# SingleRust/single-algebra

Hardware: AMD Instinct MI355X
Metric: sparse_pca_fit_transform_algorithmic_throughput (higher is better)
Workload: dtype f32

## Files before the change

single-algebra_amd/csrc/spmm_tiled.hip:

```cpp
#include <cstdio>
#include <cstdlib>
#include <cstring>

#include <rocprim/rocprim.hpp>

#include "kernels.h"
#include "spmm_dq.h"

namespace sapca {
namespace k {

namespace {

constexpr int WAVE = 64;
constexpr int LDS_TOTAL = 160 * 1024;

struct Ent { uint32_t off; float val; };
struct EntD { uint32_t off; uint32_t pad; double val; };
template <typename VT> struct EntOf { typedef Ent type; };
template <> struct EntOf<double> { typedef EntD type; };

inline int grid_for(int64_t work_items, int block, int cap = 8192) {
  int64_t g = (work_items + block - 1) / block;
  if (g < 1) g = 1;
  if (g > cap) g = cap;
  return (int)g;
}

typedef float v4f __attribute__((ext_vector_type(4)));
typedef float v4f_a4 __attribute__((ext_vector_type(4), aligned(4)));

template <int N, int THREADS>
__device__ __forceinline__ void load_regs(v4f (&r)[N], const char* src, int bytes) {
#pragma unroll
  for (int i = 0; i < N; ++i)
    r[i] = *reinterpret_cast<const v4f*>(src + min((i * THREADS + (int)threadIdx.x) * 16, bytes - 16));
}
template <int N, int THREADS>
__device__ __forceinline__ void store_regs(const v4f (&r)[N], char* dst, int capacity) {
#pragma unroll
  for (int i = 0; i < N; ++i) {
    const int b = (i * THREADS + (int)threadIdx.x) * 16;
    if ((i + 1) * THREADS * 16 <= capacity || b + 16 <= capacity) *reinterpret_cast<v4f*>(dst + b) = r[i];
  }
}

template <typename VT>
__global__ void split_reduce_kernel(const VT* __restrict__ part, int nsplit, int64_t rows, int ldo, int ncols,
                                    const VT* __restrict__ cvec, VT* __restrict__ out, int ldy) {
  const int64_t total = rows * ldo;
  int64_t i = (int64_t)blockIdx.x * blockDim.x + threadIdx.x;
  const int64_t stride = (int64_t)gridDim.x * blockDim.x;
  for (; i < total; i += stride) {
    const int j = (int)(i % ldo);
    if (j >= ncols) continue;
    VT s = 0;
    for (int sp = 0; sp < nsplit; ++sp) s += part[(int64_t)sp * total + i];
    out[(i / ldo) * ldy + j] = s - (cvec ? cvec[j] : (VT)0);
  }
}

__global__ void split_reduce_rows_kernel(const float* __restrict__ part, int nsplit, int64_t slab_stride, int64_t rows, int ldo, int ncols,
                                         float* __restrict__ out, int ldy) {
  const int64_t total = rows * ldo;
  int64_t i = (int64_t)blockIdx.x * blockDim.x + threadIdx.x;
  const int64_t stride = (int64_t)gridDim.x * blockDim.x;
  for (; i < total; i += stride) {
    const int j = (int)(i % ldo);
    if (j >= ncols) continue;
    float s = 0;
    for (int sp = 0; sp < nsplit; ++sp) s += part[(int64_t)sp * slab_stride + i];
    out[(i / ldo) * ldy + j] = s;
  }
}

#ifndef SAPCA_QWAVES
#define SAPCA_QWAVES 16
#endif
constexpr int QGROUPS = 4, QLANES = WAVE / QGROUPS, QWAVES = SAPCA_QWAVES, QTHREADS = QWAVES * WAVE;
constexpr int Q_TILE_BYTES = 80 * 1024;
constexpr int Q_MAX_TILES_RUNS = 16384;
constexpr int q_stage_bytes(int tile_bytes) { return LDS_TOTAL - tile_bytes - 1024; }
constexpr int QBLOCK_ROWS = 1024;
constexpr int Q_BLOCK_QUADS = QBLOCK_ROWS / 4;
constexpr int ENT_SLACK = 4 * WAVE;
constexpr int q_rows_per_group(int ldp) { return (ldp == 64 ? 128 : 64) / QWAVES; }
__host__ __device__ inline int q_steps(int longest) { return kOddSteps ? longest : (longest + 1) & ~1; }
__host__ __device__ inline int q_first(int wave, int nquads) { return wave * nquads / QWAVES; }

// ... 91 lines not shown
    for (int off = 1; off < WAVE; off <<= 1) {
      const uint32_t y = __shfl_up(inc, off);
      if (lane >= off) inc += y;
    }
#pragma unroll
    for (int off = WAVE / 2; off > 0; off >>= 1) raw += __shfl_xor(raw, off);
    __syncthreads();
    if (lane == WAVE - 1) wave_total[q / WAVE] = inc;
    if (lane == 0) raw_part[q / WAVE] = (uint32_t)raw;
    __syncthreads();
    for (int w = 0; w < q / WAVE; ++w) inc += wave_total[w];
    scan[q] = inc;
    __syncthreads();
    if (quad_off && q < nquads) quad_off[((int64_t)rb * Q_BLOCK_QUADS + q) * nct + ct] = inc - padded;
    if (q < QWAVES) {
      const int first_quad = q_first(q, nquads);
      wave_off[chunk * QWAVES + q] = first_quad > 0 ? scan[first_quad - 1] : 0u;
    }
    if (q == Q_BLOCK_QUADS - 1) {
      chunk_size[chunk] = inc;
      if (raw_size) {
        uint32_t total = 0;
        for (int w = 0; w < Q_BLOCK_QUADS / WAVE; ++w) total += raw_part[w];
        raw_size[chunk] = total;
      }
    }
  }
}

template <typename VT>
__global__ void __launch_bounds__(256)
quad_fill_kernel(const int64_t* __restrict__ ptr, const int32_t* __restrict__ idx, const VT* __restrict__ val,
                 int64_t rows, const int32_t* __restrict__ blk_row0, const uint32_t* __restrict__ perm, int nrb, int nct,
                 float inv_nct, int ldp_bytes, const int64_t* __restrict__ chunk_off, const uint32_t* __restrict__ quad_off,
                 typename EntOf<VT>::type* __restrict__ ent) {
  typedef typename EntOf<VT>::type E;
  extern __shared__ uint32_t cnt_all[];
  const int wave = threadIdx.x / WAVE, lane = threadIdx.x & (WAVE - 1);
  uint32_t* cnt = cnt_all + (size_t)wave * nct;
  const int64_t sp = (int64_t)blockIdx.x * 4 + wave;
  if (sp >= rows) return;
  const int64_t r = perm ? (int64_t)perm[sp] : sp;
  int lo = 0, hi = nrb;
  while (hi - lo > 1) {
    const int mid = (lo + hi) >> 1;
    if ((int64_t)blk_row0[mid] <= sp) lo = mid; else hi = mid;
  }
  const int rb = lo;
  const int lr = (int)(sp - blk_row0[rb]);
  const int qd = lr >> 2;
  const uint32_t g = (uint32_t)(lr & 3);
  const int64_t* __restrict__ coff = chunk_off + (int64_t)rb * nct;
  const uint32_t* __restrict__ qoff = quad_off + ((int64_t)rb * Q_BLOCK_QUADS + qd) * nct;
  const int64_t block_base = coff[0];
  for (int t = lane; t < nct; t += WAVE) cnt[t] = (uint32_t)(coff[t] - block_base) + qoff[t] + g;
  __builtin_amdgcn_wave_barrier();
  const int64_t e0 = ptr[r], e1 = ptr[r + 1];
  E* __restrict__ out = ent + block_base;
  for (int64_t eb = e0; eb < e1; eb += 8 * WAVE) {
    int c[8];
    VT v[8];
#pragma unroll
    for (int u = 0; u < 8; ++u) {
      const int64_t e = eb + u * WAVE + lane;
      c[u] = e < e1 ? idx[e] : -1;
      v[u] = e < e1 ? val[e] : (VT)0;
    }
#pragma unroll
    for (int u = 0; u < 8; ++u) {
      if (c[u] >= 0) {
        int i, t;
        divmod_small(c[u], nct, inv_nct, i, t);
        E x = E();
        x.off = (uint32_t)i * (uint32_t)ldp_bytes;
        x.val = v[u];
        out[atomicAdd(&cnt[t], 4u)] = x;
      }
      __builtin_amdgcn_wave_barrier();
    }
  }
}

constexpr int QF_CAP_MIN = 4096, QF_CAP_MAX = 6144;
template <typename VT>
__device__ __forceinline__ void quad_fill_staged_one(int qi, uint32_t* qf_lds, const int64_t* __restrict__ ptr, const int32_t* __restrict__ idx,
                                                     const VT* __restrict__ val, const int32_t* __restrict__ seg,
                                                     const int32_t* __restrict__ blk_row0, const uint32_t* __restrict__ perm, int nct, int cap,
                                                     float inv_nct, int ldp_bytes, const int64_t* __restrict__ chunk_off,
                                                     const uint32_t* __restrict__ quad_off, typename EntOf<VT>::type* __restrict__ ent) {
  typedef typename EntOf<VT>::type E;
  constexpr int EW = (int)sizeof(E) / 4;
  E* stage = reinterpret_cast<E*>(qf_lds);
  int64_t* gofs = reinterpret_cast<int64_t*>(qf_lds + EW * cap);
  uint32_t* lofs = qf_lds + EW * cap + 2 * nct;
  uint32_t* cnt_all = lofs + nct + 1;
  const int rb = qi / Q_BLOCK_QUADS, qd = qi % Q_BLOCK_QUADS;
  const int row0 = blk_row0[rb], nrows = blk_row0[rb + 1] - row0;
  if (4 * qd >= nrows) return;
  const int wave = threadIdx.x / WAVE, lane = threadIdx.x & (WAVE - 1);
  const int qrows = min(4, nrows - 4 * qd);
  const int64_t s0 = (int64_t)row0 + 4 * qd;
  int64_t rowof[4];
#pragma unroll
  for (int g = 0; g < 4; ++g) rowof[g] = g < qrows ? (perm ? (int64_t)perm[s0 + g] : s0 + g) : 0;
  const int64_t* __restrict__ coff = chunk_off + (int64_t)rb * nct;
  const uint32_t* __restrict__ qoff = quad_off + ((int64_t)rb * Q_BLOCK_QUADS + qd) * nct;
  for (int t = threadIdx.x; t < nct; t += 256) {
    int mx = 0;
    for (int g = 0; g < qrows; ++g) {
      const int32_t* sg = seg + rowof[g] * (nct + 1);
      mx = max(mx, sg[t + 1] - sg[t]);
    }
    lofs[t + 1] = (uint32_t)q_steps(mx) * 4u;
    gofs[t] = coff[t] + (int64_t)qoff[t];
    for (int g = 0; g < 4; ++g) cnt_all[g * nct + t] = 0;
  }
  if (threadIdx.x == 0) lofs[0] = 0;
  __syncthreads();
  if (wave == 0) {
    uint32_t carry = 0;
    for (int t0 = 0; t0 < nct; t0 += WAVE) {
      const int t = t0 + lane;
      const uint32_t v = t < nct ? lofs[t + 1] : 0u;
      uint32_t x = v;
#pragma unroll
      for (int off = 1; off < WAVE; off <<= 1) {
        const uint32_t y = __shfl_up(x, off);
        if (lane >= off) x += y;
      }
      if (t < nct) lofs[t + 1] = carry + x;
      carry += __shfl(x, WAVE - 1);
    }
  }
  __syncthreads();
  const uint32_t total = lofs[nct];
  const bool staged = total <= (uint32_t)cap;
  if (staged) {
    uint64_t* z = reinterpret_cast<uint64_t*>(stage);
    for (uint32_t i = threadIdx.x; i < total * (EW / 2); i += 256) z[i] = 0;
  } else {
    if (wave < qrows) {
      const int32_t* sg = seg + rowof[wave] * (nct + 1);
      for (int t = lane; t < nct; t += WAVE) {
        const uint32_t steps = (lofs[t + 1] - lofs[t]) / 4u;
        E* dst = ent + gofs[t];
        for (uint32_t k = (uint32_t)(sg[t + 1] - sg[t]); k < steps; ++k) dst[k * 4u + wave] = E();
      }
    } else {
      for (int t = lane; t < nct; t += WAVE) {
        const uint32_t steps = (lofs[t + 1] - lofs[t]) / 4u;
        E* dst = ent + gofs[t];
        for (uint32_t k = 0; k < steps; ++k) dst[k * 4u + wave] = E();
      }
    }
  }
  __syncthreads();
  if (wave < qrows) {
    const int64_t r = rowof[wave];
    const int64_t e0 = ptr[r], e1 = ptr[r + 1];
    uint32_t* cnt = cnt_all + (size_t)wave * nct;
    for (int64_t eb = e0; eb < e1; eb += 8 * WAVE) {
      int c[8];
      VT v[8];
#pragma unroll
      for (int u = 0; u < 8; ++u) {
        const int64_t e = eb + u * WAVE + lane;
        c[u] = e < e1 ? idx[e] : -1;
        v[u] = e < e1 ? val[e] : (VT)0;
      }
#pragma unroll
      for (int u = 0; u < 8; ++u) {
        if (c[u] >= 0) {
          int i, t;
          divmod_small(c[u], nct, inv_nct, i, t);
          E x = E();
          x.off = (uint32_t)i * (uint32_t)ldp_bytes;
          x.val = v[u];
          const uint32_t k = atomicAdd(&cnt[t], 1u);
          if (staged) stage[lofs[t] + k * 4u + (uint32_t)wave] = x;
          else ent[gofs[t] + k * 4u + (uint32_t)wave] = x;
        }
        __builtin_amdgcn_wave_barrier();
      }
    }
  }
  if (!staged) return;
  __syncthreads();
  for (int t = wave; t < nct; t += 4) {
    const uint32_t lo = lofs[t], n = lofs[t + 1] - lo;
    E* dst = ent + gofs[t];
    for (uint32_t j = lane; j < n; j += WAVE) dst[j] = stage[lo + j];
  }
}

template <typename VT>
__global__ void __launch_bounds__(256)
quad_fill_staged_kernel(const int64_t* __restrict__ ptr, const int32_t* __restrict__ idx, const VT* __restrict__ val,
                        const int32_t* __restrict__ seg, const int32_t* __restrict__ blk_row0,
                        const uint32_t* __restrict__ perm, int nct, int cap, float inv_nct,
                        int ldp_bytes, const int64_t* __restrict__ chunk_off, const uint32_t* __restrict__ quad_off,
                        typename EntOf<VT>::type* __restrict__ ent, int nquads_all) {
  extern __shared__ __attribute__((aligned(16))) uint32_t qf_lds[];
  for (int qi = blockIdx.x; qi < nquads_all; qi += gridDim.x) {
    quad_fill_staged_one<VT>(qi, qf_lds, ptr, idx, val, seg, blk_row0, perm, nct, cap, inv_nct, ldp_bytes, chunk_off, quad_off, ent);
    __syncthreads();
  }
}

__global__ void tile_index_mod_kernel(const int64_t* __restrict__ ptr, const int32_t* __restrict__ idx,
                                      const uint64_t* __restrict__ packed, int64_t rows, int nct, float inv_nct,
                                      int32_t* __restrict__ seg) {
  const int64_t total = rows * (int64_t)(nct + 1);
  int64_t o = (int64_t)blockIdx.x * blockDim.x + threadIdx.x;
  const int64_t stride = (int64_t)gridDim.x * blockDim.x;
  for (; o < total; o += stride) {
    const int64_t r = o / (nct + 1);
    const int t = (int)(o - r * (nct + 1));
    const int64_t e0 = ptr[r], e1 = ptr[r + 1];
    int64_t lo = e0, hi = e1;
    while (lo < hi) {
      const int64_t mid = (lo + hi) >> 1;
      int q, tm;
      divmod_small(packed ? (int)(packed[mid] >> 32) : idx[mid], nct, inv_nct, q, tm);
      if (tm < t) lo = mid + 1; else hi = mid;
    }
    seg[o] = (int32_t)(lo - e0);
  }
}

__global__ void at_stats_index_kernel(const int64_t* __restrict__ ptr, const uint64_t* __restrict__ packed, int64_t rows,
                                      int nct, float inv_nct, double* __restrict__ sum, double* __restrict__ sumsq,
                                      int32_t* __restrict__ seg) {
  const int lane = threadIdx.x & (WAVE - 1);
  const int64_t wave = ((int64_t)blockIdx.x * blockDim.x + threadIdx.x) / WAVE;
  const int64_t nwaves = (int64_t)gridDim.x * blockDim.x / WAVE;
  for (int64_t r = wave; r < rows; r += nwaves) {
    const int64_t e0 = ptr[r], e1 = ptr[r + 1];
    int32_t* sg = seg + r * (nct + 1);
    double a = 0, b = 0;
    int carry = -1;
    for (int64_t eb = e0; eb < e1; eb += WAVE) {
      const int64_t e = eb + lane;
      const bool valid = e < e1;
      int t = nct;
      if (valid) {
        const uint64_t pv = packed[e];
        const double v = (double)__uint_as_float((uint32_t)pv);
        a += v;
        b += v * v;
        int q;
        divmod_small((int)(pv >> 32), nct, inv_nct, q, t);
      }
      int tprev = __shfl_up(t, 1);
      if (lane == 0) tprev = carry;
      if (valid || e == e1)
        for (int tt = tprev + 1; tt <= t; ++tt) sg[tt] = (int32_t)(e - e0);
      carry = __shfl(t, WAVE - 1);
    }
    if (((e1 - e0) & (WAVE - 1)) == 0)
      for (int tt = carry + 1 + lane; tt <= nct; tt += WAVE) sg[tt] = (int32_t)(e1 - e0);
#pragma unroll
    for (int off = WAVE / 2; off > 0; off >>= 1) {
      a += __shfl_xor(a, off);
      b += __shfl_xor(b, off);
    }
    if (lane == 0) {
      sum[r] = a;
      if (sumsq) sumsq[r] = b;
    }
  }
}

__global__ void row_len_iota_kernel(const int64_t* __restrict__ ptr, int64_t rows, uint32_t* __restrict__ len,
                                    uint32_t* __restrict__ iota) {
  const int64_t r = (int64_t)blockIdx.x * blockDim.x + threadIdx.x;
  if (r < rows) {
    len[r] = (uint32_t)(ptr[r + 1] - ptr[r]);
    iota[r] = (uint32_t)r;
  }
}

__global__ void __launch_bounds__(256)
natural_quad_slots_kernel(const int64_t* __restrict__ ptr, int64_t rows, unsigned long long* __restrict__ out) {
  __shared__ unsigned long long red[4];
  unsigned long long acc = 0;
  const int64_t nq = (rows + 3) / 4;
  for (int64_t qd = (int64_t)blockIdx.x * blockDim.x + threadIdx.x; qd < nq; qd += (int64_t)gridDim.x * blockDim.x) {
    int64_t mx = 0;
// ... 846 lines not shown
          psum[(int64_t)t * n + row] = a;
          psq[(int64_t)t * n + row] = b;
        }
      }
    }
    q0 = q1;
  }
}

__global__ void __launch_bounds__(1024)
atd_stats_reduce_kernel(const double* __restrict__ psum, const double* __restrict__ psq, int64_t n, int nct,
                        double* __restrict__ sum, double* __restrict__ sumsq) {
  __shared__ double pa[16][64], pb[16][64];
  const int lane = threadIdx.x & 63, grp = threadIdx.x >> 6;
  const int64_t c = (int64_t)blockIdx.x * 64 + lane;
  const int per = (nct + 15) / 16;
  double a = 0, b = 0;
  if (c < n)
    for (int t = grp * per; t < min(nct, (grp + 1) * per); ++t) {
      a += psum[(int64_t)t * n + c];
      b += psq[(int64_t)t * n + c];
    }
  pa[grp][lane] = a;
  pb[grp][lane] = b;
  __syncthreads();
  if (grp == 0 && c < n) {
    double x = 0, y = 0;
    for (int g = 0; g < 16; ++g) {
      x += pa[g][lane];
      y += pb[g][lane];
    }
    sum[c] = x;
    sumsq[c] = y;
  }
}

}

namespace {
struct AtDirectSrc {
  const CsrView<float>* A;
  const uint16_t* cnt16;
  int64_t n2;
  DevBuf* scratch;
  double* stats;
  const uint32_t* bnd;
  int64_t nrb_nat;
  const std::vector<int32_t>* blk_nat;
  bool slots_done = false;
};

void float_blocks(int64_t n, int64_t nrb, std::vector<int32_t>& blk, float& scale) {
  scale = (float)nrb / (float)n;
  auto block_of = [&](int64_t c) { return (int64_t)(int)((float)(int)c * scale); };
  while (block_of(n - 1) > nrb - 1) scale = std::nextafterf(scale, 0.0f);
  blk.assign((size_t)nrb + 1, (int32_t)n);
  int64_t b = 0;
  blk[0] = 0;
  for (int64_t c = 0; c < n; ++c) {
    const int64_t bc = block_of(c);
    while (b < bc) blk[(size_t)++b] = (int32_t)c;
  }
  while (b < nrb) blk[(size_t)++b] = (int32_t)n;
}

int dq_block_rows(int64_t op_rows) {
  static const int dq_rows_env = dbg_env("SAPCA_DQ_BLOCK_ROWS") ? atoi(dbg_env("SAPCA_DQ_BLOCK_ROWS")) : 0;
  return dq_rows_env == 512 || dq_rows_env == 1024 ? dq_rows_env : (op_rows >= 1024 * 16 ? 1024 : 512);
}
void natural_partition(int64_t op_rows, int nct, int block_rows, int64_t& nrb, int& nsplit) {
  nrb = (op_rows + block_rows - 1) / block_rows;
  nsplit = 1;
  if (nrb >= 192) {
    nrb = round_up(nrb, 256);
  } else {
    static const int split_wgs_env = dbg_env("SAPCA_SPLIT_WGS") ? atoi(dbg_env("SAPCA_SPLIT_WGS")) : 0;
    const int64_t split_wgs = split_wgs_env > 0 ? split_wgs_env : (block_rows > 512 ? 256 : 512);
    nsplit = (int)std::min<int64_t>(nct, std::max<int64_t>(1, split_wgs / nrb));
    const int64_t nrb_fit = split_wgs / nsplit;
    if (nrb_fit >= nrb && nrb_fit <= op_rows) nrb = nrb_fit;
  }
}

inline unsigned qf_grid(int64_t nquads) {
#ifdef SAPCA_QF_WGS
  const int64_t wgs = SAPCA_QF_WGS;
#else
  const int64_t wgs = nquads;
#endif
  return (unsigned)std::max<int64_t>(1, std::min<int64_t>(nquads, wgs));
}

template <typename VT>
bool build_tiled_t(const CsrView<VT>& S, int ldp_elems, TiledOp& op, TiledBuffers& buf, hipStream_t s,
                   bool rows_tile_major, const uint64_t* packed_rows, bool seg_ready,
                   const AtDirectSrc* direct = nullptr) {
  typedef typename EntOf<VT>::type E;
  constexpr bool f32 = sizeof(VT) == 4;
  const int ldp = ldp_elems * (int)sizeof(VT) / 4;
  SAPCA_CHECK(ldp_elems == 64, SAPCA_ERR_ARG, "tiled sweep: panels must have 64 columns");
  op = TiledOp();
  if (!f32 && packed_rows) return false;
  if (S.rows == 0 || S.cols == 0 || S.nnz == 0) return false;
  const int64_t op_rows = S.rows, op_cols = S.cols;
  const int tile_bytes = Q_TILE_BYTES;
  const int tc = tile_bytes / (ldp * 4);
  if (packed_rows && !rows_tile_major) return false;
  const int nct = (int)((op_cols + tc - 1) / tc);
  const int waves = QWAVES;
  const bool dq_candidate = f32 && ldp == 64 && dbg_env("SAPCA_NO_DQ") == nullptr;
  const int block_rows = dq_candidate ? dq_block_rows(op_rows) : QWAVES * QGROUPS * q_rows_per_group(ldp);
  const int stage_cap = q_stage_bytes(tile_bytes) / (int)sizeof(E) - WAVE;
  int64_t nrb = 0;
  int nsplit = 1;
  natural_partition(op_rows, nct, block_rows, nrb, nsplit);
  if (op_cols >= (1 << 24) || nct > (rows_tile_major ? Q_MAX_TILES_RUNS : 4096)) return false;
  const float inv_nct = 1.0f / (float)nct;
  int32_t* d_seg = nullptr;
  if (direct && !(f32 && rows_tile_major && dq_candidate && tc <= 32 * ATD_MASK_WORDS && block_rows <= QBLOCK_ROWS))
    return false;
  if (!direct) {
    d_seg = buf.seg.as<int32_t>((size_t)S.rows * (nct + 1));
    if (rows_tile_major && seg_ready) {
    } else if (rows_tile_major) {
      hipLaunchKernelGGL(tile_index_mod_kernel, dim3(grid_for(S.rows * (int64_t)(nct + 1), 256, 16384)), dim3(256), 0, s,
                         S.ptr, S.idx, packed_rows, S.rows, nct, inv_nct, d_seg);
    } else {
      hipLaunchKernelGGL(tile_hist_kernel, dim3(grid_for(S.rows, 4, 8192)), dim3(256), (size_t)4 * nct * sizeof(uint32_t), s,
                         S.ptr, S.idx, S.rows, nct, inv_nct, d_seg);
    }
  }
  uint32_t* d_perm = nullptr;
  std::vector<uint32_t> sorted_len;
  bool sort_rows = dbg_env("SAPCA_NO_ROWSORT") == nullptr;
  int64_t* pinned = static_cast<int64_t*>(buf.host.ensure((size_t)(8 + 65536 + 2) * sizeof(int64_t)));
  bool speculate = false;
  bool rows_in_disorder = false;
  if (sort_rows && dbg_env("SAPCA_ROWSORT_ALWAYS") == nullptr) {
    unsigned long long* d_slots = reinterpret_cast<unsigned long long*>(buf.misc.as<int64_t>(8)) + 4;
    if (!(direct && direct->slots_done)) {
      SAPCA_HIP(hipMemsetAsync(d_slots, 0, sizeof(unsigned long long), s));
      hipLaunchKernelGGL(natural_quad_slots_kernel, dim3(grid_for((S.rows + 3) / 4, 256, 1024)), dim3(256), 0, s, S.ptr, S.rows, d_slots);
    }
    SAPCA_HIP(hipMemcpyAsync(pinned, d_slots, sizeof(unsigned long long), hipMemcpyDeviceToHost, s));
    speculate = true;
    sort_rows = false;
  }
  auto sort_now = [&] {
    uint32_t* d_len = buf.lens.as<uint32_t>((size_t)2 * S.rows);
    uint32_t* d_len_sorted = d_len + S.rows;
    uint32_t* d_iota = buf.perm.as<uint32_t>((size_t)2 * S.rows);
    d_perm = d_iota + S.rows;
    hipLaunchKernelGGL(row_len_iota_kernel, dim3(grid_for(S.rows, 256, 1 << 30)), dim3(256), 0, s, S.ptr, S.rows, d_len, d_iota);
    size_t sb = 0;
    SAPCA_HIP(rocprim::radix_sort_pairs_desc(nullptr, sb, d_len, d_len_sorted, d_iota, d_perm, (size_t)S.rows, 0u, 32u, s));
    char* tmp = static_cast<char*>(buf.tmp.ensure(sb + 256));
    SAPCA_HIP(rocprim::radix_sort_pairs_desc(tmp, sb, d_len, d_len_sorted, d_iota, d_perm, (size_t)S.rows, 0u, 32u, s));
    sorted_len.resize((size_t)S.rows);
    SAPCA_HIP(hipMemcpyAsync(sorted_len.data(), d_len_sorted, sorted_len.size() * sizeof(uint32_t), hipMemcpyDeviceToHost, s));
    SAPCA_HIP(hipStreamSynchronize(s));
  };
  if (sort_rows) sort_now();
  int tiles_per_split = 0;
  int64_t nchunks = 0, max_chunk = 0, total = 0;
  int32_t* d_blk = nullptr;
  int64_t mid_row0 = -1;
  uint8_t* d_steps = nullptr;
  uint32_t* d_wave_off = nullptr;
  uint32_t* d_quad_off = nullptr;
  int64_t* d_chunk = nullptr;
  int64_t* d_raw = nullptr;
  for (int attempt = 0;; ++attempt) {
    tiles_per_split = (nct + nsplit - 1) / nsplit;
    nsplit = (nct + tiles_per_split - 1) / tiles_per_split;
    std::vector<int32_t> blk;
    if (sort_rows) {
      const double budget = (double)S.nnz / (double)nrb;
      blk.push_back(0);
      double acc = 0;
      int in_block = 0;
      for (int64_t r = 0; r < op_rows; ++r) {
        acc += sorted_len[(size_t)r];
        ++in_block;
        const bool last = r + 1 == op_rows;
        if (last || in_block == block_rows || acc >= budget * (double)blk.size()) {
          blk.push_back((int32_t)(r + 1));
          in_block = 0;
        }
      }
      nrb = (int64_t)blk.size() - 1;
    } else if (direct && direct->bnd && nrb == direct->nrb_nat) {
      blk = *direct->blk_nat;
    } else {
      blk.resize((size_t)nrb + 1);
      for (int64_t b = 0; b <= nrb; ++b) blk[(size_t)b] = (int32_t)(op_rows * b / nrb);
    }
    nchunks = nrb * nct;
    mid_row0 = blk[(size_t)(nrb / 2)];
    d_blk = buf.blk.as<int32_t>((size_t)nrb + 1);
    d_steps = buf.steps.as<uint8_t>((size_t)nchunks * Q_BLOCK_QUADS * 2);
    d_wave_off = buf.wave_off.as<uint32_t>((size_t)nchunks * waves);
    d_quad_off = buf.run.as<uint32_t>((size_t)nchunks * Q_BLOCK_QUADS);
    d_chunk = buf.chunk_off.as<int64_t>((size_t)nchunks + 1);
    if (blk.size() <= 2 * 65536) {
      std::memcpy(pinned + 8, blk.data(), blk.size() * sizeof(int32_t));
      SAPCA_HIP(hipMemcpyAsync(d_blk, pinned + 8, blk.size() * sizeof(int32_t), hipMemcpyHostToDevice, s));
    } else {
      SAPCA_HIP(hipMemcpyAsync(d_blk, blk.data(), blk.size() * sizeof(int32_t), hipMemcpyHostToDevice, s));
    }
    if (direct) {
      d_raw = buf.rank.as<int64_t>((size_t)nchunks + 1);
      hipLaunchKernelGGL(quad_count_kernel, dim3((unsigned)(nrb * ((nct + QC_TILES - 1) / QC_TILES))), dim3(Q_BLOCK_QUADS), 0, s, d_seg, d_blk, d_perm, nct,
                         reinterpret_cast<uint16_t*>(d_steps), (uint32_t*)nullptr, d_wave_off, d_chunk, direct->cnt16, direct->n2, d_raw);
    } else
      hipLaunchKernelGGL(quad_count_kernel, dim3((unsigned)(nrb * ((nct + QC_TILES - 1) / QC_TILES))), dim3(Q_BLOCK_QUADS), 0, s, d_seg, d_blk, d_perm, nct,
                         reinterpret_cast<uint16_t*>(d_steps), d_quad_off, d_wave_off, d_chunk);
    int64_t* d_max = buf.misc.as<int64_t>(8);
    launch_small_scan(d_chunk, d_raw, nchunks, d_max, s);
    int64_t* host = pinned + 1;
    SAPCA_HIP(hipMemcpyAsync(host, d_max, (direct ? 7 : 2) * sizeof(int64_t), hipMemcpyDeviceToHost, s));
    SAPCA_HIP(hipStreamSynchronize(s));
    if (direct) rows_in_disorder = host[6] != 0;
    if (speculate) {
      speculate = false;
      if ((double)(unsigned long long)pinned[0] > 1.10 * (double)S.nnz) {
        sort_rows = true;
        sort_now();
        attempt = -1;
        continue;
      }
    }
    max_chunk = host[0];
    total = host[1];
    if (dbg_env("SAPCA_DEBUG"))
      fprintf(stderr, "sapca: build_tiled rows %lld cols %lld nrb %lld nct %d split %d max_chunk %lld (cap %d) total %lld\n",
              (long long)op_rows, (long long)op_cols, (long long)nrb, nct, nsplit,
              (long long)max_chunk, stage_cap, (long long)total);
    if (max_chunk <= stage_cap || dq_candidate) break;
    if (attempt == 3 || nrb * 2 > op_rows) return false;
    nrb *= 2;
    if (nsplit > 1) nsplit = std::max(1, nsplit / 2);
  }
  E* d_ent = reinterpret_cast<E*>(buf.ent.ensure((size_t)(total + ENT_SLACK) * sizeof(E)));
  bool aux_pending = false;
  op.rows = op_rows; op.cols = op_cols; op.ldp = ldp_elems; op.elem = (int)sizeof(VT); op.tc = tc; op.nct = nct; op.nrb = (int)nrb; op.block_rows = block_rows; op.max_chunk = max_chunk;
  op.nsplit = nsplit; op.tiles_per_split = tiles_per_split; op.total_entries = total; op.tile_bytes = tile_bytes;
  op.mid_row0 = mid_row0;
  op.blk_row0 = d_blk; op.row_perm = d_perm; op.chunk_off = d_chunk; op.wave_off = d_wave_off; op.steps = d_steps; op.ent = d_ent;
  if constexpr (f32) {
    op.valid = true;
    if (!buf.aux) {
      SAPCA_HIP(hipStreamCreateWithFlags(&buf.aux, hipStreamNonBlocking));
      SAPCA_HIP(hipEventCreateWithFlags(&buf.aux_fork, hipEventDisableTiming));
      SAPCA_HIP(hipEventCreateWithFlags(&buf.aux_join, hipEventDisableTiming));
    }
    SAPCA_HIP(hipEventRecord(buf.aux_fork, s));
    SAPCA_HIP(hipStreamWaitEvent(buf.aux, buf.aux_fork, 0));
    const bool dq_ok = dq_build_tables(op, buf, buf.aux);
    SAPCA_HIP(hipEventRecord(buf.aux_join, buf.aux));
    aux_pending = true;
    op.valid = false;
    if (!dq_ok && (block_rows > 512 || max_chunk > stage_cap)) {
      SAPCA_HIP(hipStreamWaitEvent(s, buf.aux_join, 0));
      return false;
    }
  }
  if constexpr (!f32) {
    op.valid = true;
    (void)dq_build_tables(op, buf, s);
    op.valid = false;
  }
  const int qf_cap_max = f32 ? QF_CAP_MAX : QF_CAP_MIN;
  const bool staged_fill = !rows_tile_major && dbg_env("SAPCA_FILL_DIRECT") == nullptr &&
                           (double)total <= 0.93 * qf_cap_max * ((double)op_rows / 4.0) && nct <= 768;
  static const bool qf_cap_fixed = dbg_env("SAPCA_QF_CAP_FIXED") != nullptr;
  const double quad_avg = (double)total / std::max(1.0, (double)op_rows / 4.0);
  const int qf_cap_fit = (int)std::min<int64_t>(qf_cap_max, std::max<int64_t>(2048, round_up((int64_t)(1.12 * quad_avg) + 64, 256)));
  const int qf_cap = (!f32 || qf_cap_fixed) ? ((double)total <= 0.85 * QF_CAP_MIN * ((double)op_rows / 4.0) ? QF_CAP_MIN : qf_cap_max) : qf_cap_fit;
  const bool runs_fill = rows_tile_major && nct <= Q_MAX_TILES_RUNS;
  if ((packed_rows || direct) && !runs_fill) {
    if (aux_pending) SAPCA_HIP(hipStreamWaitEvent(s, buf.aux_join, 0));
    return false;
  }
  if (staged_fill || runs_fill || direct) SAPCA_HIP(hipMemsetAsync(d_ent + total, 0, (size_t)ENT_SLACK * sizeof(E), s));
  else SAPCA_HIP(hipMemsetAsync(d_ent, 0, (size_t)(total + ENT_SLACK) * sizeof(E), s));
  if constexpr (f32) {
  if (direct) {
    const CsrView<float>& A = *direct->A;
    const size_t scan_bytes = 0;
    const bool gather = direct->bnd != nullptr && d_perm == nullptr && nrb == direct->nrb_nat && !rows_in_disorder &&
                        dbg_env("SAPCA_AT_BUCKETS") == nullptr;
    const size_t a_col = round_up((size_t)op_rows * sizeof(uint32_t), 256), a_bucket = gather ? 0 : round_up((size_t)A.nnz * sizeof(uint2), 256);
    const size_t a_part = direct->stats ? round_up((size_t)nct * op_rows * sizeof(double), 256) : 0;
    const size_t a_scan = round_up(scan_bytes + 256, 256);
    char* base = static_cast<char*>(direct->scratch->ensure(a_col + a_bucket + 2 * a_part + a_scan + (size_t)nchunks * sizeof(uint32_t) + 256));
    uint32_t* d_colmap = reinterpret_cast<uint32_t*>(base);
    uint2* d_bucket = reinterpret_cast<uint2*>(base + a_col);
    double* d_psum = direct->stats ? reinterpret_cast<double*>(base + a_col + a_bucket) : nullptr;
    double* d_psq = direct->stats ? reinterpret_cast<double*>(base + a_col + a_bucket + a_part) : nullptr;
    if (gather) {
      hipLaunchKernelGGL(atd_fill_kernel<true>, dim3((unsigned)(8 * ((nct + 7) / 8) * nrb)), dim3(ATD_THREADS), 0, s, (const uint2*)nullptr,
                         (const int64_t*)nullptr, d_blk, d_perm, nct, ldp * 4, d_chunk, d_quad_off, reinterpret_cast<const uint16_t*>(d_steps), d_ent,
                         d_psum, d_psq, op_rows, A.idx, A.val, direct->bnd, A.ptr, A.rows, tc, (int)nrb);
    } else {
      hipLaunchKernelGGL(atd_colmap_kernel, dim3((unsigned)((op_rows + 255) / 256)), dim3(256), 0, s, d_blk, (int)nrb, d_perm, op_rows,
                         d_colmap);
      uint32_t* d_cursor = reinterpret_cast<uint32_t*>(base + a_col + a_bucket + 2 * a_part + a_scan);
      SAPCA_HIP(hipMemsetAsync(d_cursor, 0, (size_t)nchunks * sizeof(uint32_t), s));
      hipLaunchKernelGGL(atd_scatter_kernel, dim3((unsigned)std::min<int64_t>(round_up((A.rows + 3) / 4, 8), 4096)), dim3(256), 0, s, A.ptr,
                         A.idx, A.val, A.rows, nct, tc, d_colmap, d_raw, d_cursor, d_bucket);
      hipLaunchKernelGGL(atd_fill_kernel<false>, dim3((unsigned)nchunks), dim3(ATD_THREADS), 0, s, d_bucket, d_raw, d_blk, d_perm, nct, ldp * 4,
                         d_chunk, d_quad_off, reinterpret_cast<const uint16_t*>(d_steps), d_ent, d_psum, d_psq, op_rows,
                         (const int32_t*)nullptr, (const float*)nullptr, (const uint32_t*)nullptr, (const int64_t*)nullptr, (int64_t)0, tc, (int)nrb);
    }
    if (direct->stats)
      hipLaunchKernelGGL(atd_stats_reduce_kernel, dim3((unsigned)((op_rows + 63) / 64)), dim3(1024), 0, s, d_psum, d_psq, op_rows, nct,
                         direct->stats, direct->stats + op_rows);
  } else if (runs_fill) {
    const int seg_lds_max = dbg_env("SAPCA_RUNS_SEG_LDS_MAX") ? atoi(dbg_env("SAPCA_RUNS_SEG_LDS_MAX")) : 1024;
    if (nct <= seg_lds_max)
      hipLaunchKernelGGL(quad_fill_runs_kernel<true>, dim3((unsigned)(nrb * Q_BLOCK_QUADS)), dim3(256),
                         (size_t)4 * (nct + 1) * sizeof(int32_t), s, S.ptr, S.idx, S.val, packed_rows, d_seg, d_blk, d_perm, nct,
                         inv_nct, ldp * 4, d_chunk, d_quad_off, d_ent);
    else
      hipLaunchKernelGGL(quad_fill_runs_kernel<false>, dim3((unsigned)(nrb * Q_BLOCK_QUADS)), dim3(256), 0, s, S.ptr, S.idx, S.val,
                         packed_rows, d_seg, d_blk, d_perm, nct, inv_nct, ldp * 4, d_chunk, d_quad_off, d_ent);
  } else if (staged_fill)
    hipLaunchKernelGGL(quad_fill_staged_kernel<float>, dim3(qf_grid((int64_t)nrb * Q_BLOCK_QUADS)), dim3(256),
                       (size_t)qf_cap * sizeof(Ent) + ((size_t)7 * nct + 1) * sizeof(uint32_t), s, S.ptr, S.idx, S.val, d_seg, d_blk,
                       d_perm, nct, qf_cap, inv_nct, ldp * 4, d_chunk, d_quad_off, d_ent, (int)(nrb * Q_BLOCK_QUADS));
  else
    hipLaunchKernelGGL(quad_fill_kernel<float>, dim3((unsigned)((S.rows + 3) / 4)), dim3(256), (size_t)4 * nct * sizeof(uint32_t), s,
                       S.ptr, S.idx, S.val, S.rows, d_blk, d_perm, (int)nrb, nct, inv_nct, ldp * 4, d_chunk, d_quad_off, d_ent);
  } else {
    if (runs_fill) {
      const int seg_lds_max = dbg_env("SAPCA_RUNS_SEG_LDS_MAX") ? atoi(dbg_env("SAPCA_RUNS_SEG_LDS_MAX")) : 1024;
      if (nct <= seg_lds_max)
        hipLaunchKernelGGL((quad_fill_runs_kernel<true, double>), dim3((unsigned)(nrb * Q_BLOCK_QUADS)), dim3(256),
                           (size_t)4 * (nct + 1) * sizeof(int32_t), s, S.ptr, S.idx, S.val, (const uint64_t*)nullptr, d_seg, d_blk, d_perm, nct,
                           inv_nct, ldp * 4, d_chunk, d_quad_off, d_ent);
      else
        hipLaunchKernelGGL((quad_fill_runs_kernel<false, double>), dim3((unsigned)(nrb * Q_BLOCK_QUADS)), dim3(256), 0, s, S.ptr, S.idx, S.val,
                           (const uint64_t*)nullptr, d_seg, d_blk, d_perm, nct, inv_nct, ldp * 4, d_chunk, d_quad_off, d_ent);
    } else if (staged_fill) {
      const size_t fill_lds = (size_t)qf_cap * sizeof(E) + ((size_t)7 * nct + 1) * sizeof(uint32_t);
      static LdsAttrState attr;
      ensure_dynamic_lds(reinterpret_cast<const void*>(&quad_fill_staged_kernel<double>), fill_lds, attr);
      hipLaunchKernelGGL(quad_fill_staged_kernel<double>, dim3(qf_grid((int64_t)nrb * Q_BLOCK_QUADS)), dim3(256), fill_lds, s, S.ptr, S.idx,
                         S.val, d_seg, d_blk, d_perm, nct, qf_cap, inv_nct, ldp * 4, d_chunk, d_quad_off, d_ent, (int)(nrb * Q_BLOCK_QUADS));
    } else
    hipLaunchKernelGGL(quad_fill_kernel<double>, dim3((unsigned)((S.rows + 3) / 4)), dim3(256), (size_t)4 * nct * sizeof(uint32_t), s,
                       S.ptr, S.idx, S.val, S.rows, d_blk, d_perm, (int)nrb, nct, inv_nct, ldp * 4, d_chunk, d_quad_off, d_ent);
  }
  SAPCA_HIP(hipGetLastError());
  if (aux_pending) SAPCA_HIP(hipStreamWaitEvent(s, buf.aux_join, 0));
  op.valid = true;
  return true;
}
}

bool build_tiled(const CsrView<float>& S, int ldp, TiledOp& op, TiledBuffers& buf, hipStream_t s,
                 bool rows_tile_major, const uint64_t* packed_rows, bool seg_ready) {
  return build_tiled_t<float>(S, ldp, op, buf, s, rows_tile_major, packed_rows, seg_ready);
}
bool build_tiled(const CsrView<double>& S, int ldp, TiledOp& op, TiledBuffers& buf, hipStream_t s, bool rows_tile_major) {
  return build_tiled_t<double>(S, ldp, op, buf, s, rows_tile_major, nullptr, false);
}

bool build_tiled_at_direct(const CsrView<float>& A, int ldp, TiledOp& op, TiledBuffers& buf, int64_t* at_ptr, double* stats,
                           DevBuf& scratch, hipStream_t s) {
  op = TiledOp();
  const bool off = dbg_env("SAPCA_AT_SORT") != nullptr;
  if (off || ldp != 64 || A.rows == 0 || A.cols == 0 || A.nnz == 0 || A.cols > ATD_MAX_COLS || A.rows >= (1 << 24)) return false;
  const int64_t m = A.rows, n = A.cols;
  const int tc = Q_TILE_BYTES / (ldp * 4);
  const int nct = tiled_tile_count(m, ldp);
  if (tc > 32 * ATD_MASK_WORDS || nct > Q_MAX_TILES_RUNS) return false;
  const int64_t n2 = round_up(n, 2);
  uint16_t* cnt16 = buf.seg.as<uint16_t>((size_t)nct * n2);
  int64_t nrb_nat = 0;
  int nsplit_nat = 1;
  natural_partition(n, nct, dq_block_rows(n), nrb_nat, nsplit_nat);
  uint32_t* bnd = nullptr;
  if (dbg_env("SAPCA_AT_BUCKETS") == nullptr && nrb_nat <= 4096) {
    try {
      bnd = buf.bounds.as<uint32_t>((size_t)(nrb_nat + 1) * (size_t)nct * tc);
    } catch (const Error&) {
      (void)hipGetLastError();
      bnd = nullptr;
    }
  }
  const size_t hist_lds = (size_t)n2 * 2;
  static LdsAttrState hist_attr;
  ensure_dynamic_lds(reinterpret_cast<const void*>(&atd_hist_kernel), hist_lds, hist_attr);
  std::vector<int32_t> blk_nat;
  float blk_scale = 0.f;
  if (bnd) float_blocks(n, nrb_nat, blk_nat, blk_scale);
  int64_t* d_disorder = buf.misc.as<int64_t>(8) + 6;
  unsigned long long* d_slots = reinterpret_cast<unsigned long long*>(buf.misc.as<int64_t>(8)) + 4;
  SAPCA_HIP(hipMemsetAsync(d_disorder, 0, sizeof(int64_t), s));
  hipLaunchKernelGGL(atd_hist_kernel, dim3((unsigned)nct), dim3((size_t)n2 * 2 > 52 * 1024 ? ATD_HIST_THREADS_WIDE : ATD_HIST_THREADS),
                     hist_lds, s, A.ptr, A.idx, m, nct, tc, n2, cnt16, blk_scale, (int)nrb_nat, bnd, d_disorder, d_slots);
  hipLaunchKernelGGL(atd_rowlen_kernel, dim3((unsigned)((n + 64) / 64)), dim3(1024), 0, s, cnt16, n, n2, nct, at_ptr, d_slots);
  launch_small_scan(at_ptr, nullptr, n, nullptr, s);
  SAPCA_HIP(hipGetLastError());
  CsrView<float> At;
  At.rows = n; At.cols = m; At.nnz = A.nnz; At.ptr = at_ptr; At.idx = nullptr; At.val = nullptr;
  AtDirectSrc src{&A, cnt16, n2, &scratch, stats, bnd, nrb_nat, &blk_nat, true};
  return build_tiled_t<float>(At, ldp, op, buf, s, true, nullptr, false, &src);
}

void at_stats_index(const int64_t* ptr, const uint64_t* packed, int64_t rows, int64_t cols, int ldp, TiledBuffers& buf,
                    double* sum, double* sumsq, hipStream_t s) {
  if (rows == 0) return;
  const int nct = tiled_tile_count(cols, ldp);
  int32_t* d_seg = buf.seg.as<int32_t>((size_t)rows * (nct + 1));
  hipLaunchKernelGGL(at_stats_index_kernel, dim3(grid_for(rows * WAVE, 256, 4096)), dim3(256), 0, s, ptr, packed, rows, nct,
                     1.0f / (float)nct, sum, sumsq, d_seg);
  SAPCA_HIP(hipGetLastError());
}

int tiled_tile_count(int64_t cols, int ldp) {
  const int tc = Q_TILE_BYTES / (ldp * 4);
  return (int)((cols + tc - 1) / tc);
}

void spmm_tiled(const TiledOp& op, const float* X, int ldx, float* Y, int ldy, int ncols, const float* cvec, DevBuf& scratch,
                hipStream_t s, PanelSource<float>* keep) {
  SAPCA_CHECK(op.valid && op.elem == 4, SAPCA_ERR_ARG, "tiled sweep: operator not built");
  SAPCA_CHECK(ldx == op.ldp || (op.ldp == 64 && ldx % 64 == 0), SAPCA_ERR_ARG,
              "tiled sweep: panel leading dimension does not match the operator's tile geometry");
  const int passes = ldx / op.ldp;
// ... 114 lines not shown
```

Measured before the change: 1336.

## Group multiple quads per workgroup in staged fill with XCD-aware block mapping

Generalizes the staged quad-fill kernel so one workgroup can process G consecutive quads (256*G threads) with a combined LDS image and a single joint prefix scan. When the combined image overflows, it falls back to one quad at a time. Blocks are remapped so contiguous items land on the same XCD, and the LDS zeroing and copy-out use 16-byte vector stores. The default group is 1, so by default only the XCD remapping and vectorized copies change; larger groups need an environment setting and add LDS pressure plus a fallback path.

```diff
diff --git a/single-algebra_amd/csrc/qf_map.h b/single-algebra_amd/csrc/qf_map.h
--- /dev/null
+++ b/single-algebra_amd/csrc/qf_map.h
@@ -0,0 +1,24 @@
+#pragma once
+
+#if defined(__HIPCC__)
+#define SAPCA_QF_HD __host__ __device__
+#else
+#define SAPCA_QF_HD
+#endif
+
+namespace sapca {
+namespace k {
+
+constexpr int QF_XCDS = 8;
+
+SAPCA_QF_HD inline int qf_items_per_xcd(int items) { return (items + QF_XCDS - 1) / QF_XCDS; }
+SAPCA_QF_HD inline int qf_virtual_blocks(int items) { return QF_XCDS * qf_items_per_xcd(items); }
+SAPCA_QF_HD inline int qf_item_of_block(int v, int items) {
+  const int per = qf_items_per_xcd(items);
+  const int x = v & (QF_XCDS - 1), j = v >> 3;
+  const int item = x * per + j;
+  return (j < per && item < items) ? item : -1;
+}
+
+}
+}
diff --git a/single-algebra_amd/csrc/spmm_tiled.hip b/single-algebra_amd/csrc/spmm_tiled.hip
--- a/single-algebra_amd/csrc/spmm_tiled.hip
+++ b/single-algebra_amd/csrc/spmm_tiled.hip
@@ -1,3 +1,4 @@
+#include <cassert>
 #include <cstdio>
 #include <cstdlib>
 #include <cstring>
@@ -5,6 +6,7 @@
 #include <rocprim/rocprim.hpp>
 
 #include "kernels.h"
+#include "qf_map.h"
 #include "spmm_dq.h"
 
 namespace sapca {
@@ -262,83 +264,99 @@
 }
 
 constexpr int QF_CAP_MIN = 4096, QF_CAP_MAX = 6144;
-template <typename VT>
-__device__ __forceinline__ void quad_fill_staged_one(int qi, uint32_t* qf_lds, const int64_t* __restrict__ ptr, const int32_t* __restrict__ idx,
-                                                     const VT* __restrict__ val, const int32_t* __restrict__ seg,
-                                                     const int32_t* __restrict__ blk_row0, const uint32_t* __restrict__ perm, int nct, int cap,
-                                                     float inv_nct, int ldp_bytes, const int64_t* __restrict__ chunk_off,
-                                                     const uint32_t* __restrict__ quad_off, typename EntOf<VT>::type* __restrict__ ent) {
+#ifndef SAPCA_QF_GROUP
+#define SAPCA_QF_GROUP 1
+#endif
+inline size_t qf_lds_bytes(int cap, int group, int nct, size_t entry_bytes) {
+  return (size_t)cap * group * entry_bytes + ((size_t)(2 + 5 * group) * nct + 1) * sizeof(uint32_t);
+}
+template <typename VT, int G>
+__device__ __forceinline__ bool quad_fill_staged_group(int rb, int q0, int nq, uint32_t* qf_lds, const int64_t* __restrict__ ptr,
+                                                       const int32_t* __restrict__ idx, const VT* __restrict__ val,
+                                                       const int32_t* __restrict__ seg, const int32_t* __restrict__ blk_row0,
+                                                       const uint32_t* __restrict__ perm, int nct, int cap, float inv_nct, int ldp_bytes,
+                                                       const int64_t* __restrict__ chunk_off, const uint32_t* __restrict__ quad_off,
+                                                       typename EntOf<VT>::type* __restrict__ ent) {
   typedef typename EntOf<VT>::type E;
   constexpr int EW = (int)sizeof(E) / 4;
+  constexpr int NT = 256 * G;
   E* stage = reinterpret_cast<E*>(qf_lds);
   int64_t* gofs = reinterpret_cast<int64_t*>(qf_lds + EW * cap);
-  uint32_t* lofs = qf_lds + EW * cap + 2 * nct;
-  uint32_t* cnt_all = lofs + nct + 1;
-  const int rb = qi / Q_BLOCK_QUADS, qd = qi % Q_BLOCK_QUADS;
+  uint32_t* qlofs = qf_lds + EW * cap + 2 * nct;
+  uint32_t* cnt_all = qlofs + G * nct + 1;
   const int row0 = blk_row0[rb], nrows = blk_row0[rb + 1] - row0;
-  if (4 * qd >= nrows) return;
   const int wave = threadIdx.x / WAVE, lane = threadIdx.x & (WAVE - 1);
-  const int qrows = min(4, nrows - 4 * qd);
-  const int64_t s0 = (int64_t)row0 + 4 * qd;
-  int64_t rowof[4];
-#pragma unroll
-  for (int g = 0; g < 4; ++g) rowof[g] = g < qrows ? (perm ? (int64_t)perm[s0 + g] : s0 + g) : 0;
+  const int wq = wave >> 2, wg = wave & 3;
+  const int nseg = nct * G;
   const int64_t* __restrict__ coff = chunk_off + (int64_t)rb * nct;
-  const uint32_t* __restrict__ qoff = quad_off + ((int64_t)rb * Q_BLOCK_QUADS + qd) * nct;
-  for (int t = threadIdx.x; t < nct; t += 256) {
+  const uint32_t* __restrict__ qoff = quad_off + ((int64_t)rb * Q_BLOCK_QUADS + q0) * nct;
+  for (int i = threadIdx.x; i < nseg; i += NT) {
+    const int t = i / G, j = i % G;
     int mx = 0;
-    for (int g = 0; g < qrows; ++g) {
-      const int32_t* sg = seg + rowof[g] * (nct + 1);
-      mx = max(mx, sg[t + 1] - sg[t]);
-    }
-    lofs[t + 1] = (uint32_t)q_steps(mx) * 4u;
-    gofs[t] = coff[t] + (int64_t)qoff[t];
-    for (int g = 0; g < 4; ++g) cnt_all[g * nct + t] = 0;
-  }
-  if (threadIdx.x == 0) lofs[0] = 0;
+    if (j < nq) {
+      const int lr0 = 4 * (q0 + j);
+      for (int g = 0; g < 4 && lr0 + g < nrows; ++g) {
+        const int64_t s0 = (int64_t)row0 + lr0 + g;
+        const int32_t* sg = seg + (perm ? (int64_t)perm[s0] : s0) * (nct + 1);
+        mx = max(mx, sg[t + 1] - sg[t]);
+      }
+    }
+    qlofs[i + 1] = (uint32_t)q_steps(mx) * 4u;
+    if (j == 0) gofs[t] = coff[t] + (int64_t)qoff[t];
+    for (int g = 0; g < 4; ++g) cnt_all[(4 * j + g) * nct + t] = 0;
+  }
+  if (threadIdx.x == 0) qlofs[0] = 0;
   __syncthreads();
   if (wave == 0) {
     uint32_t carry = 0;
-    for (int t0 = 0; t0 < nct; t0 += WAVE) {
-      const int t = t0 + lane;
-      const uint32_t v = t < nct ? lofs[t + 1] : 0u;
+    for (int i0 = 0; i0 < nseg; i0 += WAVE) {
+      const int i = i0 + lane;
+      const uint32_t v = i < nseg ? qlofs[i + 1] : 0u;
       uint32_t x = v;
 #pragma unroll
       for (int off = 1; off < WAVE; off <<= 1) {
         const uint32_t y = __shfl_up(x, off);
         if (lane >= off) x += y;
       }
-      if (t < nct) lofs[t + 1] = carry + x;
+      if (i < nseg) qlofs[i + 1] = carry + x;
       carry += __shfl(x, WAVE - 1);
     }
   }
   __syncthreads();
-  const uint32_t total = lofs[nct];
+  const uint32_t total = qlofs[nseg];
   const bool staged = total <= (uint32_t)cap;
+  if (!staged && nq > 1) return false;
+#ifdef SAPCA_DEBUG_SWITCHES
+  for (int i = threadIdx.x; i < nseg; i += NT)
+    if (i % G < nq) assert(qoff[(int64_t)(i % G) * nct + i / G] - qoff[i / G] == qlofs[i] - qlofs[i - i % G]);
+#endif
   if (staged) {
-    uint64_t* z = reinterpret_cast<uint64_t*>(stage);
-    for (uint32_t i = threadIdx.x; i < total * (EW / 2); i += 256) z[i] = 0;
-  } else {
-    if (wave < qrows) {
-      const int32_t* sg = seg + rowof[wave] * (nct + 1);
+    uint4* z = reinterpret_cast<uint4*>(stage);
+    for (uint32_t i = threadIdx.x; i < total * (uint32_t)sizeof(E) / 16u; i += NT) z[i] = make_uint4(0u, 0u, 0u, 0u);
+  } else if (wave < 4) {
+    if (4 * q0 + wave < nrows) {
+      const int64_t s0 = (int64_t)row0 + 4 * q0 + wave;
+      const int32_t* sg = seg + (perm ? (int64_t)perm[s0] : s0) * (nct + 1);
       for (int t = lane; t < nct; t += WAVE) {
-        const uint32_t steps = (lofs[t + 1] - lofs[t]) / 4u;
+        const uint32_t steps = (qlofs[t * G + 1] - qlofs[t * G]) / 4u;
         E* dst = ent + gofs[t];
         for (uint32_t k = (uint32_t)(sg[t + 1] - sg[t]); k < steps; ++k) dst[k * 4u + wave] = E();
       }
     } else {
       for (int t = lane; t < nct; t += WAVE) {
-        const uint32_t steps = (lofs[t + 1] - lofs[t]) / 4u;
+        const uint32_t steps = (qlofs[t * G + 1] - qlofs[t * G]) / 4u;
         E* dst = ent + gofs[t];
         for (uint32_t k = 0; k < steps; ++k) dst[k * 4u + wave] = E();
       }
     }
   }
   __syncthreads();
-  if (wave < qrows) {
-    const int64_t r = rowof[wave];
+  if (wq < nq && 4 * (q0 + wq) + wg < nrows) {
+    const int64_t s0 = (int64_t)row0 + 4 * (q0 + wq) + wg;
+    const int64_t r = perm ? (int64_t)perm[s0] : s0;
     const int64_t e0 = ptr[r], e1 = ptr[r + 1];
     uint32_t* cnt = cnt_all + (size_t)wave * nct;
+    const uint32_t* lofs = qlofs + wq;
     for (int64_t eb = e0; eb < e1; eb += 8 * WAVE) {
       int c[8];
       VT v[8];
@@ -357,33 +375,49 @@
           x.off = (uint32_t)i * (uint32_t)ldp_bytes;
           x.val = v[u];
           const uint32_t k = atomicAdd(&cnt[t], 1u);
-          if (staged) stage[lofs[t] + k * 4u + (uint32_t)wave] = x;
-          else ent[gofs[t] + k * 4u + (uint32_t)wave] = x;
+          if (staged) stage[lofs[t * G] + k * 4u + (uint32_t)wg] = x;
+          else ent[gofs[t] + k * 4u + (uint32_t)wg] = x;
         }
         __builtin_amdgcn_wave_barrier();
       }
     }
   }
-  if (!staged) return;
+  if (!staged) return true;
   __syncthreads();
-  for (int t = wave; t < nct; t += 4) {
-    const uint32_t lo = lofs[t], n = lofs[t + 1] - lo;
-    E* dst = ent + gofs[t];
-    for (uint32_t j = lane; j < n; j += WAVE) dst[j] = stage[lo + j];
-  }
-}
-
-template <typename VT>
-__global__ void __launch_bounds__(256)
+  constexpr uint32_t PER16 = 16u / (uint32_t)sizeof(E);
+  const uint4* img = reinterpret_cast<const uint4*>(stage);
+  for (int t = wave; t < nct; t += 4 * G) {
+    const uint32_t lo = qlofs[t * G] / PER16, n = qlofs[t * G + G] / PER16 - lo;
+    uint4* dst = reinterpret_cast<uint4*>(ent + gofs[t]);
+    for (uint32_t j = lane; j < n; j += WAVE) dst[j] = img[lo + j];
+  }
+  return true;
+}
+
+template <typename VT, int G>
+__global__ void __launch_bounds__(256 * G)
 quad_fill_staged_kernel(const int64_t* __restrict__ ptr, const int32_t* __restrict__ idx, const VT* __restrict__ val,
                         const int32_t* __restrict__ seg, const int32_t* __restrict__ blk_row0,
                         const uint32_t* __restrict__ perm, int nct, int cap, float inv_nct,
                         int ldp_bytes, const int64_t* __restrict__ chunk_off, const uint32_t* __restrict__ quad_off,
-                        typename EntOf<VT>::type* __restrict__ ent, int nquads_all) {
+                        typename EntOf<VT>::type* __restrict__ ent, int items, int gpb) {
   extern __shared__ __attribute__((aligned(16))) uint32_t qf_lds[];
-  for (int qi = blockIdx.x; qi < nquads_all; qi += gridDim.x) {
-    quad_fill_staged_one<VT>(qi, qf_lds, ptr, idx, val, seg, blk_row0, perm, nct, cap, inv_nct, ldp_bytes, chunk_off, quad_off, ent);
-    __syncthreads();
+  const int nv = qf_virtual_blocks(items);
+  for (int v = blockIdx.x; v < nv; v += gridDim.x) {
+    const int item = qf_item_of_block(v, items);
+    if (item < 0) continue;
+    const int rb = item / gpb, q0 = (item - rb * gpb) * G;
+    const int nquads = (blk_row0[rb + 1] - blk_row0[rb] + 3) >> 2;
+    if (q0 >= nquads) continue;
+    const int nq = min(G, nquads - q0);
+    for (int done = 0, n = nq; done < nq;) {
+      if (quad_fill_staged_group<VT, G>(rb, q0 + done, n, qf_lds, ptr, idx, val, seg, blk_row0, perm, nct, cap, inv_nct, ldp_bytes, chunk_off,
+                                        quad_off, ent))
+        done += n;
+      else
+        n = 1;
+      __syncthreads();
+    }
   }
 }
 
@@ -1396,13 +1430,42 @@
   }
 }
 
-inline unsigned qf_grid(int64_t nquads) {
-#ifdef SAPCA_QF_WGS
-  const int64_t wgs = SAPCA_QF_WGS;
-#else
-  const int64_t wgs = nquads;
-#endif
-  return (unsigned)std::max<int64_t>(1, std::min<int64_t>(nquads, wgs));
+inline unsigned qf_grid(int64_t items) { return (unsigned)qf_virtual_blocks((int)std::max<int64_t>(1, items)); }
+
+inline int qf_group(int nct, int cap, size_t entry_bytes) {
+  const int env = dbg_env("SAPCA_QF_GROUP") ? atoi(dbg_env("SAPCA_QF_GROUP")) : 0;
+  int group = (env == 1 || env == 2 || env == 4) ? env : SAPCA_QF_GROUP;
+  auto fits = [&](int g) {
+    const size_t bytes = qf_lds_bytes(cap, g, nct, entry_bytes);
+    return bytes <= (size_t)LDS_TOTAL && (env != 0 || ((size_t)LDS_TOTAL / bytes) * 4 * g >= 16);
+  };
+  while (group > 1 && !fits(group)) group >>= 1;
+  return group;
+}
+
+template <typename VT, int G>
+void launch_quad_fill_staged_g(const CsrView<VT>& S, const int32_t* d_seg, const int32_t* d_blk, const uint32_t* d_perm, int nct, int cap,
+                               float inv_nct, int ldp_bytes, const int64_t* d_chunk, const uint32_t* d_quad_off,
+                               typename EntOf<VT>::type* d_ent, int64_t nrb, int max_block_rows, hipStream_t s) {
+  const int gpb = ((max_block_rows + 3) / 4 + G - 1) / G;
+  const int64_t items = nrb * gpb;
+  const size_t lds = qf_lds_bytes(cap, G, nct, sizeof(typename EntOf<VT>::type));
+  if (dbg_env("SAPCA_DEBUG"))
+    fprintf(stderr, "sapca: staged fill: %d quads per workgroup, image %d entries, %lld items, LDS %zu bytes\n", G, cap * G, (long long)items, lds);
+  static LdsAttrState attr;
+  ensure_dynamic_lds(reinterpret_cast<const void*>(&quad_fill_staged_kernel<VT, G>), lds, attr);
+  hipLaunchKernelGGL((quad_fill_staged_kernel<VT, G>), dim3(qf_grid(items)), dim3(256 * G), lds, s, S.ptr, S.idx, S.val, d_seg, d_blk, d_perm,
+                     nct, cap * G, inv_nct, ldp_bytes, d_chunk, d_quad_off, d_ent, (int)items, gpb);
+}
+template <typename VT>
+void launch_quad_fill_staged(const CsrView<VT>& S, const int32_t* d_seg, const int32_t* d_blk, const uint32_t* d_perm, int nct, int cap,
+                             float inv_nct, int ldp_bytes, const int64_t* d_chunk, const uint32_t* d_quad_off,
+                             typename EntOf<VT>::type* d_ent, int64_t nrb, int max_block_rows, hipStream_t s) {
+  switch (qf_group(nct, cap, sizeof(typename EntOf<VT>::type))) {
+    case 4: launch_quad_fill_staged_g<VT, 4>(S, d_seg, d_blk, d_perm, nct, cap, inv_nct, ldp_bytes, d_chunk, d_quad_off, d_ent, nrb, max_block_rows, s); break;
+    case 2: launch_quad_fill_staged_g<VT, 2>(S, d_seg, d_blk, d_perm, nct, cap, inv_nct, ldp_bytes, d_chunk, d_quad_off, d_ent, nrb, max_block_rows, s); break;
+    default: launch_quad_fill_staged_g<VT, 1>(S, d_seg, d_blk, d_perm, nct, cap, inv_nct, ldp_bytes, d_chunk, d_quad_off, d_ent, nrb, max_block_rows, s);
+  }
 }
 
 template <typename VT>
@@ -1479,6 +1542,7 @@
   int64_t nchunks = 0, max_chunk = 0, total = 0;
   int32_t* d_blk = nullptr;
   int64_t mid_row0 = -1;
+  int max_block_rows = 0;
   uint8_t* d_steps = nullptr;
   uint32_t* d_wave_off = nullptr;
   uint32_t* d_quad_off = nullptr;
@@ -1511,6 +1575,8 @@
     }
     nchunks = nrb * nct;
     mid_row0 = blk[(size_t)(nrb / 2)];
+    max_block_rows = 0;
+    for (int64_t b = 0; b < nrb; ++b) max_block_rows = std::max(max_block_rows, (int)(blk[(size_t)b + 1] - blk[(size_t)b]));
     d_blk = buf.blk.as<int32_t>((size_t)nrb + 1);
     d_steps = buf.steps.as<uint8_t>((size_t)nchunks * Q_BLOCK_QUADS * 2);
     d_wave_off = buf.wave_off.as<uint32_t>((size_t)nchunks * waves);
@@ -1640,9 +1706,7 @@
       hipLaunchKernelGGL(quad_fill_runs_kernel<false>, dim3((unsigned)(nrb * Q_BLOCK_QUADS)), dim3(256), 0, s, S.ptr, S.idx, S.val,
                          packed_rows, d_seg, d_blk, d_perm, nct, inv_nct, ldp * 4, d_chunk, d_quad_off, d_ent);
   } else if (staged_fill)
-    hipLaunchKernelGGL(quad_fill_staged_kernel<float>, dim3(qf_grid((int64_t)nrb * Q_BLOCK_QUADS)), dim3(256),
-                       (size_t)qf_cap * sizeof(Ent) + ((size_t)7 * nct + 1) * sizeof(uint32_t), s, S.ptr, S.idx, S.val, d_seg, d_blk,
-                       d_perm, nct, qf_cap, inv_nct, ldp * 4, d_chunk, d_quad_off, d_ent, (int)(nrb * Q_BLOCK_QUADS));
+    launch_quad_fill_staged<float>(S, d_seg, d_blk, d_perm, nct, qf_cap, inv_nct, ldp * 4, d_chunk, d_quad_off, d_ent, nrb, max_block_rows, s);
   else
     hipLaunchKernelGGL(quad_fill_kernel<float>, dim3((unsigned)((S.rows + 3) / 4)), dim3(256), (size_t)4 * nct * sizeof(uint32_t), s,
                        S.ptr, S.idx, S.val, S.rows, d_blk, d_perm, (int)nrb, nct, inv_nct, ldp * 4, d_chunk, d_quad_off, d_ent);
@@ -1657,11 +1721,7 @@
         hipLaunchKernelGGL((quad_fill_runs_kernel<false, double>), dim3((unsigned)(nrb * Q_BLOCK_QUADS)), dim3(256), 0, s, S.ptr, S.idx, S.val,
                            (const uint64_t*)nullptr, d_seg, d_blk, d_perm, nct, inv_nct, ldp * 4, d_chunk, d_quad_off, d_ent);
     } else if (staged_fill) {
-      const size_t fill_lds = (size_t)qf_cap * sizeof(E) + ((size_t)7 * nct + 1) * sizeof(uint32_t);
-      static LdsAttrState attr;
-      ensure_dynamic_lds(reinterpret_cast<const void*>(&quad_fill_staged_kernel<double>), fill_lds, attr);
-      hipLaunchKernelGGL(quad_fill_staged_kernel<double>, dim3(qf_grid((int64_t)nrb * Q_BLOCK_QUADS)), dim3(256), fill_lds, s, S.ptr, S.idx,
-                         S.val, d_seg, d_blk, d_perm, nct, qf_cap, inv_nct, ldp * 4, d_chunk, d_quad_off, d_ent, (int)(nrb * Q_BLOCK_QUADS));
+      launch_quad_fill_staged<double>(S, d_seg, d_blk, d_perm, nct, qf_cap, inv_nct, ldp * 4, d_chunk, d_quad_off, d_ent, nrb, max_block_rows, s);
     } else
     hipLaunchKernelGGL(quad_fill_kernel<double>, dim3((unsigned)((S.rows + 3) / 4)), dim3(256), (size_t)4 * nct * sizeof(uint32_t), s,
                        S.ptr, S.idx, S.val, S.rows, d_blk, d_perm, (int)nrb, nct, inv_nct, ldp * 4, d_chunk, d_quad_off, d_ent);
```

New measurement: 1345 (median of 6 runs). About the same (+0.7%).
